# rafaelsoStanford/State_Policy_DiffusionModel

Measured on AMD Instinct MI355X. Metric: denoise-steps/sec (B=4096, horizon=32), higher is better.
Workload: dtype f32 (split-fp16 MFMA operands, fp32 accumulate)

## Files before the change

### include/spdm.h

```cpp
#ifndef SPDM_H
#define SPDM_H

#include <stddef.h>
#include <stdint.h>

#ifdef __cplusplus
extern "C" {
#endif

#define SPDM_NAME_MAX 64
#define SPDM_ABI_VERSION 2

typedef enum {
    SPDM_OK = 0,
    SPDM_ERR_INVALID = -1,
    SPDM_ERR_HIP = -2,
    SPDM_ERR_STATE = -3,
    SPDM_ERR_MISSING = -4,
    SPDM_ERR_NOMEM = -5
} spdm_status;

typedef enum { SPDM_DDPM = 0, SPDM_DDIM = 1 } spdm_scheduler_kind;

typedef struct spdm_handle spdm_handle;
// ... 215 lines not shown
void spdm_decoder_destroy(spdm_decoder* d);

#define SPDM_OPTIM_MAX_SEGMENTS 4
typedef struct { float* d_param; const float* d_grad; float* d_exp_avg; float* d_exp_avg_sq; uint64_t numel; } spdm_optim_segment;
size_t spdm_adam_workspace_doubles(void);
int  spdm_adam_step(int32_t device, const spdm_optim_segment* h_segments, int32_t n_segments, int64_t step,
                    float lr, float beta1, float beta2, float eps, float max_norm,
                    double* d_workspace, void* stream);
size_t spdm_adam_norm_index(void);

int  spdm_debug_geometry(int32_t M, int32_t N, int32_t K, int32_t HW, int32_t W, int32_t taps, uint32_t switches,
                         int32_t out[10]);

int  spdm_debug_whole_tiles(void);

int  spdm_op_gelu(const float* d_x, float* d_y, size_t n, void* stream);

typedef struct {
    int32_t B, H, W, K, N, taps;
    int32_t split;
    int32_t pro;
    int32_t epi;
    const float* d_src;  int32_t src_ld;
    const float* d_skip; int32_t skip_ld;  int32_t up_C;
    const float* h_weight;
    const double* d_src_stats; int32_t src_slots, src_m_tile, src_n_tiles, src_cnorm;
    const float* d_gamma; const float* d_beta;
    const double* d_skip_stats; int32_t skip_slots, skip_m_tile, skip_n_tiles, skip_cnorm;
    const float* d_skip_gamma; const float* d_skip_beta;
    const float* d_bias; const float* d_resid; int32_t resid_ld;
// ... 13 lines not shown
```

### state_policy_diffusionmodel_amd/_lib.py

```python
from __future__ import annotations

import ctypes
import os
from ctypes import POINTER, c_char_p, c_double, c_float, c_int32, c_int64, c_size_t, c_uint64, c_void_p

from .weights import TensorIndex

HERE = os.path.dirname(os.path.abspath(__file__))
LIB_PATH = os.environ.get("SPDM_LIB") or os.path.join(HERE, "libspdm_hip.so")

SPDM_DDPM, SPDM_DDIM = 0, 1
SPDM_FLAG_DEBUG_KEEP = 1
SPDM_FLAG_EXACT_FP32 = 2
SPDM_FLAG_SIMPLE_UNET = 4
SPDM_FLAG_TRAIN = 8
SPDM_FLAG_TRAIN_ATTENTION = 16
SPDM_FLAG_TRAIN_SIMPLE = 32
SPDM_ERR_INVALID = -1
SPDM_ERR_STATE = -3
ABI_VERSION = 2


class SpdmOpGemmArgs(ctypes.Structure):
    _fields_ = ([(n, c_int32) for n in ("B", "H", "W", "K", "N", "taps", "split", "pro", "epi")] +
# ... 95 lines not shown
    "spdm_encoder_update_weights": (c_int32, [c_void_p, c_void_p, c_size_t, c_void_p]),
    "spdm_decoder_create": (c_int32, [c_int32, c_void_p, c_size_t, POINTER(TensorIndex), c_int32, POINTER(c_void_p)]),
    "spdm_decoder_forward": (c_int32, [c_void_p, c_int32, c_void_p, c_void_p, c_void_p]),
    "spdm_decoder_train_loss": (c_int32, [c_void_p, c_int32, c_void_p, c_void_p, c_void_p, c_void_p, c_void_p]),
    "spdm_decoder_backward": (c_int32, [c_void_p, c_int32, c_void_p, c_void_p, c_void_p, c_void_p, c_void_p]),
    "spdm_decoder_update_weights": (c_int32, [c_void_p, c_void_p, c_size_t, c_void_p]),
    "spdm_decoder_destroy": (None, [c_void_p]),
    "spdm_adam_workspace_doubles": (c_size_t, []),
    "spdm_adam_step": (c_int32, [c_int32, POINTER(SpdmOptimSegment), c_int32, c_int64, c_float, c_float, c_float, c_float, c_float,
                                 c_void_p, c_void_p]),
    "spdm_adam_norm_index": (c_size_t, []),
    "spdm_op_gelu": (c_int32, [c_void_p, c_void_p, c_size_t, c_void_p]),
    "spdm_op_gemm": (c_int32, [POINTER(SpdmOpGemmArgs)]),
    "spdm_debug_geometry": (c_int32, [c_int32] * 6 + [ctypes.c_uint32, POINTER(c_int32 * 10)]),
    "spdm_debug_whole_tiles": (c_int32, []),
    "spdm_bench_gemm": (c_int32, [c_int32] * 12 + [POINTER(c_double)]),
}

_lib = None


def load() -> ctypes.CDLL:
    global _lib
    if _lib is not None:
        return _lib
    if not os.path.exists(LIB_PATH):
        raise RuntimeError(
            f"{LIB_PATH} not found: the HIP extension has not been built "
            "(run `python -m state_policy_diffusionmodel_amd.build`); there is no CPU fallback")
    import torch
# ... 19 lines not shown
```

### state_policy_diffusionmodel_amd/csrc/conv_wide.hip

```cpp
#include <algorithm>
#include <cstdlib>

#include "device_utils.h"

namespace spdm {

typedef float f32x16 __attribute__((ext_vector_type(16)));
typedef float f32x4 __attribute__((ext_vector_type(4)));
typedef float f32x2 __attribute__((ext_vector_type(2)));
typedef _Float16 f16x8 __attribute__((ext_vector_type(8)));
typedef _Float16 f16x2 __attribute__((ext_vector_type(2)));

namespace {

constexpr float ACT_SCALE = 16.0f;
constexpr float DESCALE = 1.0f / 2048.0f;
constexpr int CK = 32;
#ifndef WIDE_LDS_PERM
#define WIDE_LDS_PERM 1
#endif
template <bool W2, bool PIPE = false, bool WP = false> struct WidePitch { static constexpr int value = (W2 || PIPE || WP || !WIDE_LDS_PERM) ? 36 : 40; };
constexpr bool wp_active(int t, int rt) { return !((t % 3 == 0 && (rt & 3) == 0) || (t % 3 == 2 && (rt & 3) == 3)); }
constexpr int wp_first(int t) { return (t % 3 == 0) ? 1 : 0; }
constexpr int wp_next(int t, int rt, int RT) {
// ... 5 lines not shown
    int n = 0;
    for (int tt = 0; tt < t; ++tt)
        for (int r = 0; r < RT; ++r) n += wp_active(tt, r) ? 1 : 0;
    for (int r = 0; r < rt; ++r) n += wp_active(t, r) ? 1 : 0;
    return n;
}
#ifndef WIDE_STAGE_GROUP
#define WIDE_STAGE_GROUP 1
#endif
#ifndef WIDE_DB
#define WIDE_DB 0
#endif
#ifndef WIDE_EARLY
#define WIDE_EARLY 0
#endif
#ifndef WIDE_NH
#define WIDE_NH 2
#endif

__device__ __forceinline__ f32x2 split2(float a, float b) {
    unsigned h, l;
    split_pair_f16(a * ACT_SCALE, b * ACT_SCALE, h, l);
    return f32x2{__builtin_bit_cast(float, h), __builtin_bit_cast(float, l)};
}

template <int NT, int PRO, bool W2, int RT, int WN, bool PIPE, bool TWO = false, int WP = 0, bool G2 = false, int WH = 0>
#ifndef WIDE_MINB
#define WIDE_MINB 2
#endif
__global__ __launch_bounds__(256, WIDE_MINB) void conv3x3_wide_kernel(const GemmArgs a, const int epi_slots, const int NS) {
    constexpr int WM = 4 / WN;
    constexpr int CT = 2 * NT;
    constexpr int RW = RT * 16;
    constexpr int NTHR = 256;
    constexpr int RP = NTHR / 8;
    constexpr int M_T = WM * RW, N_T = WN * NT * 32;
    constexpr bool WHOLE = (WH != 0);
    constexpr bool ONE = (WH == 2);
    constexpr int APASS = WHOLE ? M_T / RP : (M_T + 18 + RP - 1) / RP;
    constexpr int FAR = (W2 || WP) ? 4 : 3;
    constexpr int FBR = (NT == 2) ? 2 : 3;
    constexpr int PH = 3 * NT;
    constexpr int BB = (APASS <= 9) ? 7 : (APASS <= 10) ? 6 : 5;
    static_assert(APASS * BB <= 64, "sample-index packing");
    static_assert(!W2 || NT == 2, "the width-2 variant exists for 128-wide tiles");
    static_assert(RT == 8 || (RT == 4 && NT == 2 && !W2), "64-row waves only in the tap-pair loop");
    static_assert(WN == 2 || (WN == 1 && RT == 4), "the 4 x 1 wave arrangement uses 64-row waves");
    static_assert(!TWO || (!PIPE && PRO != PRO_GN_GELU), "two-source input: first conv of a block, plain hand-over");
    static_assert(WP == 0 || WP == 4 || WP == 8, "row permutation for width-4 or width-8 maps");
    static_assert(!WP || (NT == 2 && WN == 2 && !W2 && !PIPE), "row permutation: 128-wide tiles");
    static_assert((16 + 4 * (WP == 8 ? 7 : 6)) % 4 == 0, "A ring phase");
    static_assert(WP != 8 || RT == 8, "width-8 maps: one 128-row block per wave");
    constexpr bool WP8 = (WP == 8);
    constexpr int NI8 = (M_T + 18 + 6) / 8 + 1;
    static_assert(!G2 || (NT == 2 && RT == 4 && !W2 && !PIPE && !WP && !WIDE_DB), "two chunks per hand-over: the plain tap loop, 64 rows per wave");
    static_assert(!WHOLE || (!G2 && !WIDE_DB && !WIDE_EARLY), "whole-sample staging: not in the hand-over experiments");
    extern __shared__ __attribute__((aligned(16))) float smem[];
// ... 24 lines not shown
    float* Abuf = smem;
    float* Awr = smem + (DB ? QZ * LDK : 0);
    float* smean = smem + ((DB || G2) ? 2 : 1) * QZ * LDK;
    float* srstd = smean + NS;

#ifdef SPDM_DIAG
    const bool stamping = (a.debug & DBG_STAMP) && a.stamps != nullptr && tid == 0;
#define WIDE_STAMP(k_) if (stamping) a.stamps[(size_t)bid * 8 + (k_)] = (unsigned long long)__builtin_amdgcn_s_memtime();
    if (stamping) {
        a.stamps[(size_t)bid * 8 + 0] = (unsigned long long)__builtin_amdgcn_s_memrealtime();
        a.stamps[(size_t)bid * 8 + 6] = (unsigned long long)__builtin_amdgcn_s_getreg(63492);
        a.stamps[(size_t)bid * 8 + 7] = (unsigned long long)__builtin_amdgcn_s_getreg(63508);
    }
    const bool dbg_no_mfma = (a.debug & DBG_NO_MFMA) != 0, dbg_no_wload = (a.debug & DBG_NO_WLOAD) != 0;
    const bool dbg_no_aload = (a.debug & DBG_NO_ALOAD) != 0;
#else
#define WIDE_STAMP(k_)
    constexpr bool dbg_no_mfma = false, dbg_no_wload = false, dbg_no_aload = false;
#endif
    WIDE_STAMP(1)
    const int zrow = WP8 ? 8 * NI8 : QA;
    if (tid < LDK) { Abuf[zrow * LDK + tid] = 0.f; Awr[zrow * LDK + tid] = 0.f; }
    if (G2 && tid < LDK) Abuf[(QZ + QA) * LDK + tid] = 0.f;

    constexpr bool pro = (PRO != PRO_NONE);
    constexpr bool pro_gelu = (PRO == PRO_GN_GELU);
    int bh_first = 0;
    float mu1 = 0.f, rs1 = 1.f;
    const int lhw = WHOLE ? __builtin_ctz((unsigned)HW) : 0;
    if constexpr (pro && ONE) {
        sample_mean_rstd(a.pro_stats, m0 / HW, mu1, rs1);
        mu1 = __builtin_bit_cast(float, __builtin_amdgcn_readfirstlane(__builtin_bit_cast(int, mu1)));
        rs1 = __builtin_bit_cast(float, __builtin_amdgcn_readfirstlane(__builtin_bit_cast(int, rs1)));
// ... 55 lines not shown
    const size_t wtap = (size_t)(N >> 4) * 2 * 256;

    f32x4 acc[RT][CT];
#pragma unroll
    for (int rt = 0; rt < RT; ++rt)
#pragma unroll
        for (int ct = 0; ct < CT; ++ct) acc[rt][ct] = f32x4{0.f, 0.f, 0.f, 0.f};

    f32x4 areg[APASS];
    f32x4 g4r = {1.f, 1.f, 1.f, 1.f}, b4r = {0.f, 0.f, 0.f, 0.f};

    int srow_o = srow_t;
#ifdef WIDE_NO_OPAQUE
#define WIDE_OPAQUE_ROW
#else
#define WIDE_OPAQUE_ROW if constexpr (PRO != PRO_NONE && RT == 8) asm volatile("" : "+v"(srow_o));
#endif
#define WIDE_LOAD_A(chunk_) WIDE_LOAD_A_(chunk_, areg, g4r, b4r, ident)
#define WIDE_STAGE_A() WIDE_STAGE_A_(areg, g4r, b4r, ident, Awr)
#define WIDE_LOAD_A_(chunk_, areg_, g4r_, b4r_, ident_)                                              \
    {                                                                                                \
        WIDE_OPAQUE_ROW                                                                              \
        const bool first_ = !TWO || (chunk_) < nc0;                                                  \
        const int cc_ = (TWO && !first_) ? (chunk_) - nc0 : (chunk_);       \
        const float* ab_ = (first_ ? abase : abase1) + cc_ * CK;                                     \
        const int ld_ = first_ ? a.src_ld : a.skip_ld;                                               \
        _Pragma("unroll") for (int p_ = 0; p_ < APASS; ++p_) {                                      \
            const int mc_ = WHOLE ? m0 + p_ * RP + srow_o : min(max(m0 - halo + p_ * RP + srow_o, 0), M - 1); \
            areg_[p_] = *reinterpret_cast<const f32x4*>(ab_ + (size_t)mc_ * ld_);                     \
        }                                                                                            \
        if (pro) {                                                                                   \
// ... 30 lines not shown
                }                                                                                    \
            }                                                                                        \
            if (!WHOLE && !((avalid >> p_) & 1u)) v_ = f32x4{0.f, 0.f, 0.f, 0.f};                       \
            const f32x2 p0_ = split2(v_.x, v_.y), p1_ = split2(v_.z, v_.w);                          \
            {                    \
                const int q_ = p_ * RP + srow_o;                                                     \
                float* row_ = (dst_) + (WHOLE ? (WP8 ? (q_ & 7) * NI8 + (q_ >> 3) : q_) : WP8 ? (q_ < QA ? ((q_ + 7) & 7) * NI8 + ((q_ + 7) >> 3) : 8 * NI8 + 1) : min(q_, QA + 1)) * LDK; \
                *reinterpret_cast<f32x2*>(row_ + c4 * 2) = f32x2{p0_.x, p1_.x};              \
                *reinterpret_cast<f32x2*>(row_ + 16 + c4 * 2) = f32x2{p0_.y, p1_.y};         \
            }                                                                                        \
            if (pro && (p_ % WIDE_STAGE_GROUP) == WIDE_STAGE_GROUP - 1) __builtin_amdgcn_sched_barrier(0);    \
        }                                                                                            \
    }
#define WIDE_LOAD_B(slot_, chunk_, tap_, cp_)                                                        \
    if (!dbg_no_wload) {                                                                             \
        const float* p_ = wfl + (size_t)((tap_) * nchunks + (chunk_)) * wtap + (cp_) * 1024;         \
        _Pragma("unroll") for (int c_ = 0; c_ < 2; ++c_) {                                          \
            fb[slot_][c_][0] = *reinterpret_cast<const f16x8*>(p_ + c_ * 512);                       \
            fb[slot_][c_][1] = *reinterpret_cast<const f16x8*>(p_ + c_ * 512 + 256);                 \
        }                                                                                            \
    }
#define WIDE_LOAD_FA(slot_, tap_, shift_, rt_)                                                       \
    {                                                                                                \
        const unsigned mb_ = (am[(rt_) / 3] >> (9 * ((rt_) % 3) + (tap_))) & 1u;                     \
        const int o_ = mb_ ? aoff0 + WIDE_LDSOFF(rt_) * LDK + (shift_) : zoff;                       \
        fa[slot_][0] = *reinterpret_cast<const f16x8*>(Abuf + o_);                                   \
        fa[slot_][1] = *reinterpret_cast<const f16x8*>(Abuf + o_ + 16);                              \
    }
#define WIDE_STEP(fas_, fbs_, rt_, ct0_)                                                             \
    if (!dbg_no_mfma) {                                                                              \
        acc[rt_][(ct0_)] = __builtin_amdgcn_mfma_f32_16x16x32_f16(fa[fas_][0], fb[fbs_][0][0], acc[rt_][(ct0_)], 0, 0, 0);         \
        acc[rt_][(ct0_) + 1] = __builtin_amdgcn_mfma_f32_16x16x32_f16(fa[fas_][0], fb[fbs_][1][0], acc[rt_][(ct0_) + 1], 0, 0, 0); \
        acc[rt_][(ct0_)] = __builtin_amdgcn_mfma_f32_16x16x32_f16(fa[fas_][0], fb[fbs_][0][1], acc[rt_][(ct0_)], 0, 0, 0);         \
        acc[rt_][(ct0_) + 1] = __builtin_amdgcn_mfma_f32_16x16x32_f16(fa[fas_][0], fb[fbs_][1][1], acc[rt_][(ct0_) + 1], 0, 0, 0); \
        acc[rt_][(ct0_)] = __builtin_amdgcn_mfma_f32_16x16x32_f16(fa[fas_][1], fb[fbs_][0][0], acc[rt_][(ct0_)], 0, 0, 0);         \
        acc[rt_][(ct0_) + 1] = __builtin_amdgcn_mfma_f32_16x16x32_f16(fa[fas_][1], fb[fbs_][1][0], acc[rt_][(ct0_) + 1], 0, 0, 0); \
    }

    const int nrows = (kc1 - kc0) * 3;
    f16x8 fa[FAR][2], fb[FBR][2][2];
#define WIDE_SHIFT(kr_, dwi_) (WP8 ? (((dwi_) - 1) * NI8 + ((kr_) - 1)) * LDK : (((kr_) - 1) * W + ((dwi_) - 1)) * LDK)

    if constexpr (!W2 && NT == 2 && !(WP && RT == 8)) {
        f16x8 fbt[2][4][2], fat[2][2];
#define TAP_LOAD_B(slot_, chunk_, tap_)                                                              \
        if (!dbg_no_wload) {                                                                         \
            const float* p_ = wfl + (size_t)((tap_) * nchunks + (chunk_)) * wtap;                    \
            _Pragma("unroll") for (int c_ = 0; c_ < 4; ++c_) {                                      \
                fbt[slot_][c_][0] = *reinterpret_cast<const f16x8*>(p_ + c_ * 512);                  \
                fbt[slot_][c_][1] = *reinterpret_cast<const f16x8*>(p_ + c_ * 512 + 256);            \
            }                                                                                        \
        }
#define TAP_LOAD_FA(slot_, tap_, shift_, rt_)                                                        \
        {                                                                                            \
            const unsigned mb_ = (am[(rt_) / 3] >> (9 * ((rt_) % 3) + (tap_))) & 1u;                 \
            const int o_ = mb_ ? aoff0 + WIDE_ROWOFF(rt_) * LDK + (shift_) : zoff;                   \
            fat[slot_][0] = *reinterpret_cast<const f16x8*>(Abuf + o_);                              \
            fat[slot_][1] = *reinterpret_cast<const f16x8*>(Abuf + o_ + 16);                         \
        }
        const int TAPS = a.taps;
        const bool t3 = (TAPS == 3);
#define TAP_SHIFT(tap_) (t3 ? ((tap_) - 1) * W * LDK : (((tap_) / 3 - 1) * W + ((tap_) - ((tap_) / 3) * 3 - 1)) * LDK)
// ... 282 lines not shown
                tap = ntap;
                chunk = nchunk;
            }
        }
        }
#undef TAP_LOAD_B
#undef TAP_LOAD_FA
#undef TAP_SHIFT
#undef TAP_BIT
    } else if constexpr (WP) {
#define WP_PLUS(i_) (WP8 ? (i_) : (i_) + (i_) / 3)
#define WP_MINUS(i_) (WP8 ? (i_) + 1 : (i_) + (i_) / 3 + 1)
        constexpr int WS = WP8 ? 7 : 6;
        constexpr int Q1 = 16 + 2 * WS, Q2 = 16 + 4 * WS;
        WIDE_LOAD_B(0, kc0, 1, 0)
        WIDE_LOAD_A(kc0)
        WIDE_STAGE_A()
        __syncthreads();
        WIDE_STAMP(2)
        WIDE_LOAD_FA(0, 1, WIDE_SHIFT(0, 1), 0)
        WIDE_LOAD_FA(1, 1, WIDE_SHIFT(0, 1), 1)
        int chunk = kc0, kr = 0;
        for (int r = 0; r < nrows; ++r) {
            int nkr = kr + 1, nchunk = chunk;
            if (nkr == 3) { nkr = 0; nchunk = chunk + 1; }
            const bool have_next = (r + 1 < nrows);
            const bool next_A = have_next && (nkr == 0);
            const int bkr = have_next ? nkr : kr, bchunk = have_next ? nchunk : chunk;
#pragma unroll
            for (int cp = 0; cp < 2; ++cp) {
                if (cp == 0) { WIDE_LOAD_B(1, chunk, kr * 3 + 1, 1) } else { WIDE_LOAD_B(0, chunk, kr * 3 + 2, 0) }
#pragma unroll
                for (int rt = 0; rt < RT; ++rt) {
                    const int q = cp * 8 + rt;
                    if (q + 2 < 16) { WIDE_LOAD_FA((q + 2) % FAR, kr * 3 + 1, WIDE_SHIFT(kr, 1), (q + 2) % 8) }
                    else { WIDE_LOAD_FA((q + 2) % FAR, kr * 3 + 2, WIDE_SHIFT(kr, 2), WP_PLUS(q + 2 - 16)) }
                    __builtin_amdgcn_sched_barrier(0);
                    WIDE_STEP(q % FAR, cp, rt, cp * 2)
                    __builtin_amdgcn_sched_barrier(0);
                }
            }
#pragma unroll
            for (int cp = 0; cp < 2; ++cp) {
                if (cp == 0) { WIDE_LOAD_B(1, chunk, kr * 3 + 2, 1) } else { WIDE_LOAD_B(0, chunk, kr * 3, 0) }
#pragma unroll
                for (int i = 0; i < WS; ++i) {
                    const int q = 16 + cp * WS + i;
                    if (q + 2 < Q1) { WIDE_LOAD_FA((q + 2) % FAR, kr * 3 + 2, WIDE_SHIFT(kr, 2), WP_PLUS((q + 2 - 16) % WS)) }
                    else { WIDE_LOAD_FA((q + 2) % FAR, kr * 3, WIDE_SHIFT(kr, 0), WP_MINUS(q + 2 - Q1)) }
                    __builtin_amdgcn_sched_barrier(0);
                    WIDE_STEP(q % FAR, cp, WP_PLUS(i), cp * 2)
                    __builtin_amdgcn_sched_barrier(0);
                }
            }
#pragma unroll
            for (int cp = 0; cp < 2; ++cp) {
                if (cp == 0) { WIDE_LOAD_B(1, chunk, kr * 3, 1) } else { WIDE_LOAD_B(0, bchunk, bkr * 3 + 1, 0) }
#pragma unroll
                for (int i = 0; i < WS; ++i) {
                    const int q = Q1 + cp * WS + i;
                    if (q + 2 < Q2) { WIDE_LOAD_FA((q + 2) % FAR, kr * 3, WIDE_SHIFT(kr, 0), WP_MINUS((q + 2 - Q1) % WS)) }
                    else if (have_next && !next_A) { WIDE_LOAD_FA((q + 2) % FAR, nkr * 3 + 1, WIDE_SHIFT(nkr, 1), q + 2 - Q2) }
                    __builtin_amdgcn_sched_barrier(0);
                    WIDE_STEP(q % FAR, cp, WP_MINUS(i), cp * 2)
                    __builtin_amdgcn_sched_barrier(0);
                }
            }
            if (next_A) {
                WIDE_LOAD_A(nchunk)
                __syncthreads();
                WIDE_STAGE_A()
                __syncthreads();
                WIDE_LOAD_FA(0, 1, WIDE_SHIFT(0, 1), 0)
                WIDE_LOAD_FA(1, 1, WIDE_SHIFT(0, 1), 1)
            }
            kr = nkr;
            chunk = nchunk;
        }
#undef WP_PLUS
// ... 35 lines not shown
                }
            }
            if (next_A) {
                WIDE_LOAD_A(nchunk)
                __syncthreads();
                WIDE_STAGE_A()
                __syncthreads();
                WIDE_LOAD_FA(0, 0, WIDE_SHIFT(0, 0), 0)
                WIDE_LOAD_FA(1, 0, WIDE_SHIFT(0, 0), 1)
            }
            kr = nkr;
            chunk = nchunk;
        }
    } else {
        WIDE_LOAD_B(0, kc0, 1, 0)
        WIDE_LOAD_A(kc0)
        WIDE_STAGE_A()
        __syncthreads();
        WIDE_STAMP(2)
        WIDE_LOAD_FA(0, 1, WIDE_SHIFT(0, 1), 0)
        WIDE_LOAD_FA(1, 1, WIDE_SHIFT(0, 1), 1)
        int chunk = kc0, kr = 0;
        for (int r = 0; r < nrows; ++r) {
            int nkr = kr + 1, nchunk = chunk;
            if (nkr == 3) { nkr = 0; nchunk = chunk + 1; }
            const bool have_next = (r + 1 < nrows);
            const bool next_A = have_next && (nkr == 0);
            const int bkr = have_next ? nkr : kr, bchunk = have_next ? nchunk : chunk;
#pragma unroll
            for (int cp = 0; cp < 2; ++cp) {
                if (cp == 0) { WIDE_LOAD_B(1, chunk, kr * 3 + 1, 1) } else { WIDE_LOAD_B(0, chunk, kr * 3 + 2, 0) }
#pragma unroll
                for (int rt = 0; rt < RT; ++rt) {
                    const int q = cp * 8 + rt;
                    if (q + 2 < 16) { WIDE_LOAD_FA((q + 2) % FAR, kr * 3 + 1, WIDE_SHIFT(kr, 1), (q + 2) % 8) }
                    else { WIDE_LOAD_FA((q + 2) % FAR, kr * 3 + 2, WIDE_SHIFT(kr, 2), 2 * (q + 2 - 16)) }
                    __builtin_amdgcn_sched_barrier(0);
                    WIDE_STEP(q % FAR, cp, rt, cp * 2)
                    __builtin_amdgcn_sched_barrier(0);
                }
            }
#pragma unroll
            for (int cp = 0; cp < 2; ++cp) {
                if (cp == 0) { WIDE_LOAD_B(1, chunk, kr * 3 + 2, 1) } else { WIDE_LOAD_B(0, chunk, kr * 3, 0) }
#pragma unroll
                for (int i = 0; i < 4; ++i) {
                    const int q = 16 + cp * 4 + i;
                    if (q + 2 < 24) { WIDE_LOAD_FA((q + 2) % FAR, kr * 3 + 2, WIDE_SHIFT(kr, 2), 2 * ((q + 2 - 16) % 4)) }
                    else { WIDE_LOAD_FA((q + 2) % FAR, kr * 3, WIDE_SHIFT(kr, 0), 2 * (q + 2 - 24) + 1) }
                    __builtin_amdgcn_sched_barrier(0);
                    WIDE_STEP(q % FAR, cp, 2 * i, cp * 2)
                    __builtin_amdgcn_sched_barrier(0);
                }
            }
#pragma unroll
            for (int cp = 0; cp < 2; ++cp) {
                if (cp == 0) { WIDE_LOAD_B(1, chunk, kr * 3, 1) } else { WIDE_LOAD_B(0, bchunk, bkr * 3 + 1, 0) }
#pragma unroll
                for (int i = 0; i < 4; ++i) {
                    const int q = 24 + cp * 4 + i;
                    if (q + 2 < 32) { WIDE_LOAD_FA((q + 2) % FAR, kr * 3, WIDE_SHIFT(kr, 0), 2 * ((q + 2 - 24) % 4) + 1) }
                    else if (have_next && !next_A) { WIDE_LOAD_FA((q + 2) % FAR, nkr * 3 + 1, WIDE_SHIFT(nkr, 1), q + 2 - 32) }
                    __builtin_amdgcn_sched_barrier(0);
                    WIDE_STEP(q % FAR, cp, 2 * i + 1, cp * 2)
                    __builtin_amdgcn_sched_barrier(0);
                }
            }
            if (next_A) {
                WIDE_LOAD_A(nchunk)
                __syncthreads();
                WIDE_STAGE_A()
                __syncthreads();
                WIDE_LOAD_FA(0, 1, WIDE_SHIFT(0, 1), 0)
                WIDE_LOAD_FA(1, 1, WIDE_SHIFT(0, 1), 1)
            }
            kr = nkr;
            chunk = nchunk;
        }
    }
#undef WIDE_LOAD_A
#undef WIDE_STAGE_A
#undef WIDE_LOAD_B
#undef WIDE_LOAD_FA
#undef WIDE_STEP
#undef WIDE_SHIFT
    WIDE_STAMP(3)
    __syncthreads();

#pragma unroll
    for (int rt = 0; rt < RT; ++rt)
#pragma unroll
        for (int ct = 0; ct < CT; ++ct) acc[rt][ct] *= DESCALE;

    const int rb4 = PERM ? ((0x1320 >> (4 * kg)) & 0xF) : kg;
    constexpr int NH = W2 ? 2 : WP ? RT / 4 : WIDE_NH;
    constexpr int HROWS = M_T / NH;
    const bool partial_out = ksp > 1;
// ... 102 lines not shown
#pragma unroll 4
        for (int p = 0; p < HROWS / RPP; ++p) {
            const int lr = p * RPP + r0;
            const int row = m0 + (lr / (RW / NH)) * RW + h * (RW / NH) + lr % (RW / NH);
            if (row < M) {
                const f32x4 v = *reinterpret_cast<const f32x4*>(otile + lr * N_T + c4o * 4);
                *reinterpret_cast<f32x4*>(dstp + (size_t)row * dst_ld + n0 + c4o * 4) = v;
            }
        }
    }
    WIDE_STAMP(5)
#undef WIDE_STAMP
#undef WIDE_ROWOFF
}

template <int NT, int PRO, bool W2 = false, int RT = 8, int WN = 2, bool PIPE = false, bool TWO = false, int WP = 0, bool G2 = false, int WH = 0>
hipError_t launch_wide_cfg(const GemmArgs& a, const GemmGeom& g, hipStream_t s) {
    constexpr int M_T = (4 / WN) * RT * 16, N_T = WN * 32 * NT, NTHR = 256;
    constexpr int APASS = WH ? M_T / 32 : (M_T + 18 + 31) / 32, NSMAX = (APASS <= 9) ? 128 : (APASS <= 10) ? 64 : 32;
    if (WH && (M_T % a.HW != 0 || a.M % M_T != 0 || (WH == 2 && a.HW != M_T))) return hipErrorInvalidValue;
    const int halo = WH ? 0 : a.W + 1;
    const int QA = M_T + 2 * halo;
    const int NS = (((QA - 1) / a.HW + 2) + 3) & ~3;
    if (NS > NSMAX || g.m_tile != M_T || g.n_tile != N_T) return hipErrorInvalidValue;
    constexpr bool DB = PIPE || (WIDE_DB && (NT == 2) && !W2);
    constexpr int LDK = WidePitch<W2, PIPE, (WP != 0) || G2>::value;
    if (PIPE && a.taps != 9) return hipErrorInvalidValue;
    if (WP && (a.taps != 9 || a.W != WP || a.HW % (4 * WP) != 0)) return hipErrorInvalidValue;
    const int QZ = (WP == 8) ? 8 * ((M_T + 18 + 6) / 8 + 1) + 2 : QA + 2;
    size_t lds = (size_t)(((DB || G2) ? 2 : 1) * QZ * LDK + 2 * NS) * sizeof(float);
    lds = std::max(lds, (size_t)((M_T / (W2 ? 2 : WP ? RT / 4 : WIDE_NH)) * N_T + (M_T / 4) * WN * 2) * sizeof(float));
    if (lds > 160 * 1024) return hipErrorInvalidValue;
    auto kern = conv3x3_wide_kernel<NT, PRO, W2, RT, WN, PIPE, TWO, WP, G2, WH>;
    if (hipError_t e = allow_full_lds(reinterpret_cast<const void*>(kern)); e != hipSuccess) return e;
    const int n_mtiles = (a.M + M_T - 1) / M_T;
    if (a.ksplit > 1 && a.K % 64 != 0) return hipErrorInvalidValue;
    if (a.route) *a.route = GemmRoute{ROUTE_WIDE, WP == 4 ? VAR_WP4 : WP == 8 ? VAR_WP8 : W2 ? VAR_W2 : PIPE ? VAR_PIPE : G2 ? VAR_G2 : VAR_PLAIN, M_T, N_T, WH};
    hipLaunchKernelGGL(kern, dim3(n_mtiles * g.n_tiles * std::max(a.ksplit, 1)), dim3(NTHR), lds, s, a, g.slots, NS);
    return hipGetLastError();
}

template <int MODES, int NT, int PRO, bool W2 = false, int RT = 8, int WN = 2, bool PIPE = false, bool TWO = false, int WP = 0>
hipError_t launch_wide_sel(const GemmArgs& a, const GemmGeom& g, hipStream_t s) {
    constexpr int M_T = (4 / WN) * RT * 16;
    const bool whole = !(a.sw & SW_NO_WHOLE_TILES) && M_T % a.HW == 0 && a.M % M_T == 0;
    if constexpr ((MODES & 2) != 0 && PRO != PRO_NONE)
        if (whole && a.HW == M_T) return launch_wide_cfg<NT, PRO, W2, RT, WN, PIPE, TWO, WP, false, 2>(a, g, s);
    if constexpr ((MODES & 1) != 0)
        if (whole) return launch_wide_cfg<NT, PRO, W2, RT, WN, PIPE, TWO, WP, false, 1>(a, g, s);
    return launch_wide_cfg<NT, PRO, W2, RT, WN, PIPE, TWO, WP, false, 0>(a, g, s);
}

}

static bool wide_w2(const GemmArgs& a) { return a.W == 2 && a.taps == 9 && !(a.sw & SW_NO_W2); }

bool conv_wide_supported(const GemmArgs& a, const GemmGeom& g) {
    const bool common = a.split && a.wgt_frag != nullptr && a.W >= 1 && a.W <= 8 && (a.HW & 3) == 0 && a.M % a.HW == 0 &&
                        a.epi == EPI_STATS && a.row_stats == nullptr && a.K % CK == 0 &&
                        (a.debug & ~(DBG_STAMP | DBG_NO_MFMA | DBG_NO_WLOAD | DBG_NO_ALOAD)) == 0 && !(a.sw & SW_NO_WIDE);
    if (!common || a.pro > PRO_GN_GELU) return false;
    if (a.skip != nullptr) {
        if (a.pro == PRO_GN_GELU || a.up_C <= 0 || a.up_C >= a.K || a.up_C % CK != 0 || g.n_tile != 128 || a.skip_ld % 4 != 0 ||
            a.skip_ld < a.K - a.up_C || a.src_ld < a.up_C) return false;
    }
    if (a.ksplit > 1 && a.K % 64 != 0) return false;
    if ((g.m_tile + 2 * (a.W + 1) - 1) / a.HW + 2 > 128) return false;
    if (g.m_tile == 128)
        return g.n_tile == 128 && (a.taps == 9 || (a.taps == 3 && a.W == 1)) && a.K % 64 == 0 && !(a.sw & SW_NO_WIDE128);
    if (g.m_tile != 256) return false;
    if (a.taps == 3) return false;
    if (a.taps != 9 || !(g.n_tile == 128 || g.n_tile == 64)) return false;
    if (wide_w2(a)) return g.n_tile == 128 && (a.HW & 7) == 0;
    if (g.n_tile == 128 && a.K % 64 != 0) return false;
    return true;
// ... 88 lines not shown
```

### state_policy_diffusionmodel_amd/csrc/kernels.h

```cpp
#pragma once
#include <hip/hip_runtime.h>
#include <stdint.h>
#include <mutex>
#include <set>
#include <utility>
#include <vector>

namespace spdm {

inline hipError_t allow_full_lds(const void* kern) {
    static std::mutex mu;
    static std::set<std::pair<int, const void*>> done;
    int dev = 0;
    hipError_t e = hipGetDevice(&dev);
    if (e != hipSuccess) return e;
    std::lock_guard<std::mutex> lk(mu);
    if (done.count({dev, kern})) return hipSuccess;
    e = hipFuncSetAttribute(kern, hipFuncAttributeMaxDynamicSharedMemorySize, (int)(160 * 1024));
    if (e == hipSuccess) done.insert({dev, kern});
    return e;
}

struct StatsRef {
    const double* p;
// ... 28 lines not shown
        {"SPDM_FILM_LOCAL", SW_FILM_LOCAL}, {"SPDM_PIN_GEOMETRY", SW_PIN_GEOMETRY},
        {"SPDM_NO_WP4", SW_NO_WP4}, {"SPDM_G2", SW_G2}, {"SPDM_NO_WP8", SW_NO_WP8},
        {"SPDM_NO_SA_HEAD", SW_NO_SA_HEAD}, {"SPDM_SA_HEAD", SW_SA_HEAD}, {"SPDM_NO_REG64", SW_NO_REG64},
        {"SPDM_NO_SA_CROP", SW_NO_SA_CROP}, {"SPDM_NO_SA_OUTC", SW_NO_SA_OUTC}, {"SPDM_NO_WHOLE_TILES", SW_NO_WHOLE_TILES}};
    *n = (int)(sizeof(t) / sizeof(t[0]));
    return t;
}
unsigned switches_from_env();
int spdm_tune(int idx, int dflt);

enum { PRO_NONE = 0, PRO_GN = 1, PRO_GN_GELU = 2, PRO_POOL = 3, PRO_UPCAT = 4 };
enum { EPI_STATS = 0, EPI_BIAS = 1, EPI_BIAS_GELU = 2, EPI_BIAS_RESID = 3, EPI_PLAIN = 4 };

enum { ROUTE_GEMM = 0, ROUTE_SKINNY = 1, ROUTE_REG = 2, ROUTE_WIDE = 3 };
enum { VAR_PLAIN = 0, VAR_W2 = 1, VAR_WP4 = 2, VAR_WP8 = 3, VAR_PIPE = 4, VAR_G2 = 5 };
struct GemmRoute { int kernel, variant, m_tile, n_tile, whole; };

struct GemmArgs {
    const float* src;  int src_ld;
    const float* wgt;
    int split;
    const float* wgt_frag;
    float* dst;        int dst_ld;
    int M, K, N;
    int geom_M;
    int taps;
    int H, W, HW;
    int pro;  StatsRef pro_stats;  const float* pro_gamma;  const float* pro_beta;
    int up_C;  const float* skip;  int skip_ld;  StatsRef skip_stats;  const float* skip_gamma;  const float* skip_beta;
    int epi;  double* epi_stats;   const float* bias;  const float* resid;  int resid_ld;
    double* row_stats;
    int ksplit;  float* partial;
    unsigned sw;
    int debug;
    unsigned long long* stamps;
    GemmRoute* route;
};
enum { DBG_NO_MFMA = 1, DBG_NO_WLOAD = 2, DBG_NO_GELU = 4, DBG_NO_STORE = 8, DBG_NO_ALOAD = 16, DBG_PP = 64, DBG_STAMP = 128 };

struct GemmGeom {
    int m_tile, n_tile, n_tiles;
    int slots;
    int ksplit;
    int skinny;
    int reg;
    int st_m_tile, st_n_tiles;
};
GemmGeom gemm_geometry(int M, int N, int K, int HW, int W, int taps, int split, unsigned sw, bool stats_epi = false);
GemmGeom gemm_geometry(const GemmArgs& a);
constexpr size_t SPLITK_WORKSPACE_BYTES = (size_t)48 << 20;
__host__ __device__ inline int combine_rows(int HW, int N) {
    int r = HW;
    while ((r & 1) == 0 && (long long)r * N > 2048) r >>= 1;
// ... 283 lines not shown
```

### state_policy_diffusionmodel_amd/csrc/spdm_api.hip

```cpp
#include <hip/hip_runtime.h>

#include <algorithm>
#include <cmath>
#include <cstdarg>
#include <cstdio>
#include <cstdlib>
#include <cstring>
#include <map>
#include <set>
#include <string>
#include <vector>

#include "../../include/spdm.h"
#include "kernels.h"

using namespace spdm;

static thread_local char g_err[512] = "";
static int fail(int code, const char* fmt, ...) {
    va_list ap;
    va_start(ap, fmt);
    vsnprintf(g_err, sizeof(g_err), fmt, ap);
    va_end(ap);
    return code;
// ... 3369 lines not shown
    out[6] = g.st_m_tile; out[7] = g.st_n_tiles;
    out[8] = stats_slots_reserved(HW, N, g.slots);
    out[9] = combine_rows(HW, N);
    return SPDM_OK;
}

extern "C" int spdm_op_gelu(const float* d_x, float* d_y, size_t n, void* stream) {
    if (!d_x || !d_y || n == 0) return fail(SPDM_ERR_INVALID, "bad argument");
    HIP_TRY(launch_gelu(d_x, d_y, n, (hipStream_t)stream));
    if (!stream) HIP_TRY(hipStreamSynchronize(nullptr));
    return SPDM_OK;
}

static int g_op_gemm_whole = -1;
extern "C" int spdm_debug_whole_tiles(void) { return g_op_gemm_whole; }

extern "C" int spdm_op_gemm(spdm_op_gemm_args* p) {
    g_op_gemm_whole = -1;
    if (!p) return fail(SPDM_ERR_INVALID, "op_gemm: null argument");
    spdm_op_gemm_args& q = *p;
    for (int i = 0; i < 10; ++i) q.out[i] = -1;
    const int HW = q.H * q.W;
    if (q.B <= 0 || q.H <= 0 || q.W <= 0 || q.K <= 0 || q.N <= 0) return fail(SPDM_ERR_INVALID, "op_gemm: empty shape");
    if (!(q.taps == 9 || q.taps == 3 || q.taps == 1)) return fail(SPDM_ERR_INVALID, "op_gemm: taps must be 9, 3 or 1");
    if (q.taps == 3 && q.W != 1) return fail(SPDM_ERR_INVALID, "op_gemm: 3-tap convolutions need W == 1");
    if (q.taps == 1 && HW != 1) return fail(SPDM_ERR_INVALID, "op_gemm: a Linear layer has H == W == 1 (B = rows)");
    if (q.taps != 1 && q.W > 8) return fail(SPDM_ERR_INVALID, "op_gemm: maps wider than 8");
    if (q.K % 32 != 0 || q.N % 64 != 0) return fail(SPDM_ERR_INVALID, "op_gemm: K %% 32 == 0 and N %% 64 == 0 required (K %d, N %d)", q.K, q.N);
    if (q.pro < PRO_NONE || q.pro > PRO_UPCAT || q.epi < EPI_STATS || q.epi > EPI_PLAIN) return fail(SPDM_ERR_INVALID, "op_gemm: unknown pro / epi");
    if (!q.d_src || !q.d_dst || !q.h_weight) return fail(SPDM_ERR_INVALID, "op_gemm: src, dst and weight are required");
    if (q.dst_ld < q.N || q.dst_ld % 4 || q.src_ld % 4) return fail(SPDM_ERR_INVALID, "op_gemm: bad leading dimension");
    const bool fused = q.pro == PRO_POOL || q.pro == PRO_UPCAT, two = !fused && q.d_skip != nullptr;
    if (q.src_ld < ((fused && q.pro == PRO_UPCAT) || two ? q.up_C : q.K)) return fail(SPDM_ERR_INVALID, "op_gemm: src_ld too small");
// ... 44 lines not shown
    AffineSrc src{q.d_src, q.src_ld}, skip{q.d_skip, q.skip_ld};
    if (q.d_src_stats)
        src = AffineSrc{q.d_src, q.src_ld, ref(q.d_src_stats, q.src_slots, q.src_m_tile, q.src_n_tiles, src_rows,
                                               q.src_cnorm > 0 ? q.src_cnorm : src_c), q.d_gamma, q.d_beta};
    if (q.d_skip_stats)
        skip = AffineSrc{q.d_skip, q.skip_ld, ref(q.d_skip_stats, q.skip_slots, q.skip_m_tile, q.skip_n_tiles, HW,
                                                  q.skip_cnorm > 0 ? q.skip_cnorm : q.K - q.up_C), q.d_skip_gamma, q.d_skip_beta};
    const int pro = (two && q.d_skip_stats) ? PRO_GN : q.pro;
    GemmArgs a = gemm_args(M, M, q.H, q.W, q.K, q.N, q.taps, split, sw, dp, pro, src, q.up_C, skip, dw,
                           dwf, q.d_dst, q.dst_ld, q.epi, q.epi == EPI_STATS ? q.d_stats : nullptr, q.d_bias,
                           q.d_resid, q.resid_ld, q.d_row_stats);
    if (fused && !gemm_takes_fused_source(a))
        return fail(SPDM_ERR_INVALID, "op_gemm: this launch does not take a fused source (the plan materialises it)");
    if (two && !gemm_takes_two_sources(a))
        return fail(SPDM_ERR_INVALID, "op_gemm: this launch does not take a two-source input (the plan concatenates)");
    GemmRoute r{-1, -1, -1, -1, 0};
    a.route = &r;
    if (q.epi == EPI_STATS) HIP_TRY(hipMemset(q.d_stats, 0xff, (size_t)q.B * g.slots * 2 * sizeof(double)));
    if (q.d_row_stats) HIP_TRY(hipMemset(q.d_row_stats, 0xff, (size_t)M * g.n_tiles * 2 * sizeof(double)));
    const hipError_t el = launch_gemm(a, nullptr);
    const hipError_t es = hipDeviceSynchronize();
    if (el != hipSuccess)
        return fail(el == hipErrorInvalidValue && r.kernel < 0 ? SPDM_ERR_INVALID : SPDM_ERR_HIP,
                    "op_gemm: launch_gemm failed (%s) %s; device: %s", hipGetErrorString(el),
                    r.kernel < 0 ? "before any kernel was dispatched (a host-side shape contract)" : "after a kernel was dispatched",
                    hipGetErrorString(es));
    if (es != hipSuccess) return fail(SPDM_ERR_HIP, "op_gemm: %s", hipGetErrorString(es));
    g_op_gemm_whole = (r.kernel == ROUTE_WIDE) ? r.whole : 0;
    q.out[0] = r.kernel; q.out[1] = r.variant; q.out[2] = r.m_tile; q.out[3] = r.n_tile; q.out[4] = g.ksplit;
    q.out[5] = two ? 1 : 0; q.out[6] = fused ? 1 : 0; q.out[7] = g.slots; q.out[8] = g.st_m_tile; q.out[9] = g.st_n_tiles;
    return SPDM_OK;
}
```

Measured before the change: 506,500.

## Deepen wide-conv weight-fragment ring to three slots for whole-tile W2/WP kernels

Adds a template parameter that lets the wide 3x3 conv kernel keep a three-slot ring of weight (B) fragments instead of two, so weight loads are issued two half-phases ahead of their MFMA use. The aim is to hide global/L2 latency on weight fetches. The deeper ring is enabled by default only for whole-tile, RT=8, width-2 or permuted-pitch variants. It costs extra VGPRs per thread, which may lower occupancy or cause spills. A debug flag that pins weight loads to one hot address and a route query for the ring depth are also added.

```diff
diff --git a/include/spdm.h b/include/spdm.h
--- a/include/spdm.h
+++ b/include/spdm.h
@@ -253,6 +253,8 @@
 
 int  spdm_debug_whole_tiles(void);
 
+int  spdm_debug_weight_ring(void);
+
 int  spdm_op_gelu(const float* d_x, float* d_y, size_t n, void* stream);
 
 typedef struct {
diff --git a/state_policy_diffusionmodel_amd/_lib.py b/state_policy_diffusionmodel_amd/_lib.py
--- a/state_policy_diffusionmodel_amd/_lib.py
+++ b/state_policy_diffusionmodel_amd/_lib.py
@@ -133,6 +133,7 @@
     "spdm_op_gemm": (c_int32, [POINTER(SpdmOpGemmArgs)]),
     "spdm_debug_geometry": (c_int32, [c_int32] * 6 + [ctypes.c_uint32, POINTER(c_int32 * 10)]),
     "spdm_debug_whole_tiles": (c_int32, []),
+    "spdm_debug_weight_ring": (c_int32, []),
     "spdm_bench_gemm": (c_int32, [c_int32] * 12 + [POINTER(c_double)]),
 }
 
diff --git a/state_policy_diffusionmodel_amd/csrc/conv_wide.hip b/state_policy_diffusionmodel_amd/csrc/conv_wide.hip
--- a/state_policy_diffusionmodel_amd/csrc/conv_wide.hip
+++ b/state_policy_diffusionmodel_amd/csrc/conv_wide.hip
@@ -43,6 +43,9 @@
 #ifndef WIDE_EARLY
 #define WIDE_EARLY 0
 #endif
+#ifndef WIDE_FBR
+#define WIDE_FBR 3
+#endif
 #ifndef WIDE_NH
 #define WIDE_NH 2
 #endif
@@ -53,7 +56,7 @@
     return f32x2{__builtin_bit_cast(float, h), __builtin_bit_cast(float, l)};
 }
 
-template <int NT, int PRO, bool W2, int RT, int WN, bool PIPE, bool TWO = false, int WP = 0, bool G2 = false, int WH = 0>
+template <int NT, int PRO, bool W2, int RT, int WN, bool PIPE, bool TWO = false, int WP = 0, bool G2 = false, int WH = 0, int BR = 2>
 #ifndef WIDE_MINB
 #define WIDE_MINB 2
 #endif
@@ -68,8 +71,10 @@
     constexpr bool ONE = (WH == 2);
     constexpr int APASS = WHOLE ? M_T / RP : (M_T + 18 + RP - 1) / RP;
     constexpr int FAR = (W2 || WP) ? 4 : 3;
-    constexpr int FBR = (NT == 2) ? 2 : 3;
+    constexpr int FBR = (NT == 2) ? BR : 3;
+    constexpr int FBD = (NT == 2) ? FBR - 1 : 1;
     constexpr int PH = 3 * NT;
+    static_assert(BR == 2 || BR == 3, "B ring: two or three phases (6 phases per kernel row: slots stay compile-time)");
     constexpr int BB = (APASS <= 9) ? 7 : (APASS <= 10) ? 6 : 5;
     static_assert(APASS * BB <= 64, "sample-index packing");
     static_assert(!W2 || NT == 2, "the width-2 variant exists for 128-wide tiles");
@@ -124,9 +129,10 @@
     }
     const bool dbg_no_mfma = (a.debug & DBG_NO_MFMA) != 0, dbg_no_wload = (a.debug & DBG_NO_WLOAD) != 0;
     const bool dbg_no_aload = (a.debug & DBG_NO_ALOAD) != 0;
+    const bool dbg_hot_wload = (a.debug & DBG_HOT_WLOAD) != 0;
 #else
 #define WIDE_STAMP(k_)
-    constexpr bool dbg_no_mfma = false, dbg_no_wload = false, dbg_no_aload = false;
+    constexpr bool dbg_no_mfma = false, dbg_no_wload = false, dbg_no_aload = false, dbg_hot_wload = false;
 #endif
     WIDE_STAMP(1)
     const int zrow = WP8 ? 8 * NI8 : QA;
@@ -212,7 +218,7 @@
 #ifdef WIDE_NO_OPAQUE
 #define WIDE_OPAQUE_ROW
 #else
-#define WIDE_OPAQUE_ROW if constexpr (PRO != PRO_NONE && RT == 8) asm volatile("" : "+v"(srow_o));
+#define WIDE_OPAQUE_ROW if constexpr ((PRO != PRO_NONE || (W2 && BR == 3)) && RT == 8) asm volatile("" : "+v"(srow_o));
 #endif
 #define WIDE_LOAD_A(chunk_) WIDE_LOAD_A_(chunk_, areg, g4r, b4r, ident)
 #define WIDE_STAGE_A() WIDE_STAGE_A_(areg, g4r, b4r, ident, Awr)
@@ -273,12 +279,24 @@
     }
 #define WIDE_LOAD_B(slot_, chunk_, tap_, cp_)                                                        \
     if (!dbg_no_wload) {                                                                             \
-        const float* p_ = wfl + (size_t)((tap_) * nchunks + (chunk_)) * wtap + (cp_) * 1024;         \
+        const float* p_ = wfl + (size_t)(dbg_hot_wload ? kc0 : (tap_) * nchunks + (chunk_)) * wtap + (cp_) * 1024; \
         _Pragma("unroll") for (int c_ = 0; c_ < 2; ++c_) {                                          \
             fb[slot_][c_][0] = *reinterpret_cast<const f16x8*>(p_ + c_ * 512);                       \
             fb[slot_][c_][1] = *reinterpret_cast<const f16x8*>(p_ + c_ * 512 + 256);                 \
         }                                                                                            \
     }
+#define WIDE_AHEAD_CENTRE(cp_)                                                                       \
+    if constexpr (FBD == 1) { if ((cp_) == 0) { WIDE_LOAD_B(1, chunk, kr * 3 + 1, 1) } else { WIDE_LOAD_B(0, chunk, kr * 3 + 2, 0) } } \
+    else { if ((cp_) == 0) { WIDE_LOAD_B(2, chunk, kr * 3 + 2, 0) } else { WIDE_LOAD_B(0, chunk, kr * 3 + 2, 1) } }
+#define WIDE_AHEAD_PLUS(cp_)                                                                         \
+    if constexpr (FBD == 1) { if ((cp_) == 0) { WIDE_LOAD_B(1, chunk, kr * 3 + 2, 1) } else { WIDE_LOAD_B(0, chunk, kr * 3, 0) } } \
+    else { if ((cp_) == 0) { WIDE_LOAD_B(1, chunk, kr * 3, 0) } else { WIDE_LOAD_B(2, chunk, kr * 3, 1) } }
+#define WIDE_AHEAD_MINUS(cp_)                                                                        \
+    if constexpr (FBD == 1) { if ((cp_) == 0) { WIDE_LOAD_B(1, chunk, kr * 3, 1) } else { WIDE_LOAD_B(0, bchunk, bkr * 3 + 1, 0) } } \
+    else { if ((cp_) == 0) { WIDE_LOAD_B(0, bchunk, bkr * 3 + 1, 0) } else { WIDE_LOAD_B(1, bchunk, bkr * 3 + 1, 1) } }
+#define WIDE_SLOT_CENTRE(cp_) (cp_)
+#define WIDE_SLOT_PLUS(cp_) (FBR == 2 ? (cp_) : 2 - 2 * (cp_))
+#define WIDE_SLOT_MINUS(cp_) (FBR == 2 ? (cp_) : 1 + (cp_))
 #define WIDE_LOAD_FA(slot_, tap_, shift_, rt_)                                                       \
     {                                                                                                \
         const unsigned mb_ = (am[(rt_) / 3] >> (9 * ((rt_) % 3) + (tap_))) & 1u;                     \
@@ -304,7 +322,7 @@
         f16x8 fbt[2][4][2], fat[2][2];
 #define TAP_LOAD_B(slot_, chunk_, tap_)                                                              \
         if (!dbg_no_wload) {                                                                         \
-            const float* p_ = wfl + (size_t)((tap_) * nchunks + (chunk_)) * wtap;                    \
+            const float* p_ = wfl + (size_t)(dbg_hot_wload ? kc0 : (tap_) * nchunks + (chunk_)) * wtap; \
             _Pragma("unroll") for (int c_ = 0; c_ < 4; ++c_) {                                      \
                 fbt[slot_][c_][0] = *reinterpret_cast<const f16x8*>(p_ + c_ * 512);                  \
                 fbt[slot_][c_][1] = *reinterpret_cast<const f16x8*>(p_ + c_ * 512 + 256);            \
@@ -617,6 +635,7 @@
         constexpr int WS = WP8 ? 7 : 6;
         constexpr int Q1 = 16 + 2 * WS, Q2 = 16 + 4 * WS;
         WIDE_LOAD_B(0, kc0, 1, 0)
+        if constexpr (FBD == 2) { WIDE_LOAD_B(1, kc0, 1, 1) }
         WIDE_LOAD_A(kc0)
         WIDE_STAGE_A()
         __syncthreads();
@@ -632,40 +651,40 @@
             const int bkr = have_next ? nkr : kr, bchunk = have_next ? nchunk : chunk;
 #pragma unroll
             for (int cp = 0; cp < 2; ++cp) {
-                if (cp == 0) { WIDE_LOAD_B(1, chunk, kr * 3 + 1, 1) } else { WIDE_LOAD_B(0, chunk, kr * 3 + 2, 0) }
+                WIDE_AHEAD_CENTRE(cp)
 #pragma unroll
                 for (int rt = 0; rt < RT; ++rt) {
                     const int q = cp * 8 + rt;
                     if (q + 2 < 16) { WIDE_LOAD_FA((q + 2) % FAR, kr * 3 + 1, WIDE_SHIFT(kr, 1), (q + 2) % 8) }
                     else { WIDE_LOAD_FA((q + 2) % FAR, kr * 3 + 2, WIDE_SHIFT(kr, 2), WP_PLUS(q + 2 - 16)) }
                     __builtin_amdgcn_sched_barrier(0);
-                    WIDE_STEP(q % FAR, cp, rt, cp * 2)
+                    WIDE_STEP(q % FAR, WIDE_SLOT_CENTRE(cp), rt, cp * 2)
                     __builtin_amdgcn_sched_barrier(0);
                 }
             }
 #pragma unroll
             for (int cp = 0; cp < 2; ++cp) {
-                if (cp == 0) { WIDE_LOAD_B(1, chunk, kr * 3 + 2, 1) } else { WIDE_LOAD_B(0, chunk, kr * 3, 0) }
+                WIDE_AHEAD_PLUS(cp)
 #pragma unroll
                 for (int i = 0; i < WS; ++i) {
                     const int q = 16 + cp * WS + i;
                     if (q + 2 < Q1) { WIDE_LOAD_FA((q + 2) % FAR, kr * 3 + 2, WIDE_SHIFT(kr, 2), WP_PLUS((q + 2 - 16) % WS)) }
                     else { WIDE_LOAD_FA((q + 2) % FAR, kr * 3, WIDE_SHIFT(kr, 0), WP_MINUS(q + 2 - Q1)) }
                     __builtin_amdgcn_sched_barrier(0);
-                    WIDE_STEP(q % FAR, cp, WP_PLUS(i), cp * 2)
+                    WIDE_STEP(q % FAR, WIDE_SLOT_PLUS(cp), WP_PLUS(i), cp * 2)
                     __builtin_amdgcn_sched_barrier(0);
                 }
             }
 #pragma unroll
             for (int cp = 0; cp < 2; ++cp) {
-                if (cp == 0) { WIDE_LOAD_B(1, chunk, kr * 3, 1) } else { WIDE_LOAD_B(0, bchunk, bkr * 3 + 1, 0) }
+                WIDE_AHEAD_MINUS(cp)
 #pragma unroll
                 for (int i = 0; i < WS; ++i) {
                     const int q = Q1 + cp * WS + i;
                     if (q + 2 < Q2) { WIDE_LOAD_FA((q + 2) % FAR, kr * 3, WIDE_SHIFT(kr, 0), WP_MINUS((q + 2 - Q1) % WS)) }
                     else if (have_next && !next_A) { WIDE_LOAD_FA((q + 2) % FAR, nkr * 3 + 1, WIDE_SHIFT(nkr, 1), q + 2 - Q2) }
                     __builtin_amdgcn_sched_barrier(0);
-                    WIDE_STEP(q % FAR, cp, WP_MINUS(i), cp * 2)
+                    WIDE_STEP(q % FAR, WIDE_SLOT_MINUS(cp), WP_MINUS(i), cp * 2)
                     __builtin_amdgcn_sched_barrier(0);
                 }
             }
@@ -731,6 +750,7 @@
         }
     } else {
         WIDE_LOAD_B(0, kc0, 1, 0)
+        if constexpr (FBD == 2) { WIDE_LOAD_B(1, kc0, 1, 1) }
         WIDE_LOAD_A(kc0)
         WIDE_STAGE_A()
         __syncthreads();
@@ -746,40 +766,40 @@
             const int bkr = have_next ? nkr : kr, bchunk = have_next ? nchunk : chunk;
 #pragma unroll
             for (int cp = 0; cp < 2; ++cp) {
-                if (cp == 0) { WIDE_LOAD_B(1, chunk, kr * 3 + 1, 1) } else { WIDE_LOAD_B(0, chunk, kr * 3 + 2, 0) }
+                WIDE_AHEAD_CENTRE(cp)
 #pragma unroll
                 for (int rt = 0; rt < RT; ++rt) {
                     const int q = cp * 8 + rt;
                     if (q + 2 < 16) { WIDE_LOAD_FA((q + 2) % FAR, kr * 3 + 1, WIDE_SHIFT(kr, 1), (q + 2) % 8) }
                     else { WIDE_LOAD_FA((q + 2) % FAR, kr * 3 + 2, WIDE_SHIFT(kr, 2), 2 * (q + 2 - 16)) }
                     __builtin_amdgcn_sched_barrier(0);
-                    WIDE_STEP(q % FAR, cp, rt, cp * 2)
+                    WIDE_STEP(q % FAR, WIDE_SLOT_CENTRE(cp), rt, cp * 2)
                     __builtin_amdgcn_sched_barrier(0);
                 }
             }
 #pragma unroll
             for (int cp = 0; cp < 2; ++cp) {
-                if (cp == 0) { WIDE_LOAD_B(1, chunk, kr * 3 + 2, 1) } else { WIDE_LOAD_B(0, chunk, kr * 3, 0) }
+                WIDE_AHEAD_PLUS(cp)
 #pragma unroll
                 for (int i = 0; i < 4; ++i) {
                     const int q = 16 + cp * 4 + i;
                     if (q + 2 < 24) { WIDE_LOAD_FA((q + 2) % FAR, kr * 3 + 2, WIDE_SHIFT(kr, 2), 2 * ((q + 2 - 16) % 4)) }
                     else { WIDE_LOAD_FA((q + 2) % FAR, kr * 3, WIDE_SHIFT(kr, 0), 2 * (q + 2 - 24) + 1) }
                     __builtin_amdgcn_sched_barrier(0);
-                    WIDE_STEP(q % FAR, cp, 2 * i, cp * 2)
+                    WIDE_STEP(q % FAR, WIDE_SLOT_PLUS(cp), 2 * i, cp * 2)
                     __builtin_amdgcn_sched_barrier(0);
                 }
             }
 #pragma unroll
             for (int cp = 0; cp < 2; ++cp) {
-                if (cp == 0) { WIDE_LOAD_B(1, chunk, kr * 3, 1) } else { WIDE_LOAD_B(0, bchunk, bkr * 3 + 1, 0) }
+                WIDE_AHEAD_MINUS(cp)
 #pragma unroll
                 for (int i = 0; i < 4; ++i) {
                     const int q = 24 + cp * 4 + i;
                     if (q + 2 < 32) { WIDE_LOAD_FA((q + 2) % FAR, kr * 3, WIDE_SHIFT(kr, 0), 2 * ((q + 2 - 24) % 4) + 1) }
                     else if (have_next && !next_A) { WIDE_LOAD_FA((q + 2) % FAR, nkr * 3 + 1, WIDE_SHIFT(nkr, 1), q + 2 - 32) }
                     __builtin_amdgcn_sched_barrier(0);
-                    WIDE_STEP(q % FAR, cp, 2 * i + 1, cp * 2)
+                    WIDE_STEP(q % FAR, WIDE_SLOT_MINUS(cp), 2 * i + 1, cp * 2)
                     __builtin_amdgcn_sched_barrier(0);
                 }
             }
@@ -798,6 +818,12 @@
 #undef WIDE_LOAD_A
 #undef WIDE_STAGE_A
 #undef WIDE_LOAD_B
+#undef WIDE_AHEAD_CENTRE
+#undef WIDE_AHEAD_PLUS
+#undef WIDE_AHEAD_MINUS
+#undef WIDE_SLOT_CENTRE
+#undef WIDE_SLOT_PLUS
+#undef WIDE_SLOT_MINUS
 #undef WIDE_LOAD_FA
 #undef WIDE_STEP
 #undef WIDE_SHIFT
@@ -930,7 +956,7 @@
 #undef WIDE_ROWOFF
 }
 
-template <int NT, int PRO, bool W2 = false, int RT = 8, int WN = 2, bool PIPE = false, bool TWO = false, int WP = 0, bool G2 = false, int WH = 0>
+template <int NT, int PRO, bool W2 = false, int RT = 8, int WN = 2, bool PIPE = false, bool TWO = false, int WP = 0, bool G2 = false, int WH = 0, int BR = 2>
 hipError_t launch_wide_cfg(const GemmArgs& a, const GemmGeom& g, hipStream_t s) {
     constexpr int M_T = (4 / WN) * RT * 16, N_T = WN * 32 * NT, NTHR = 256;
     constexpr int APASS = WH ? M_T / 32 : (M_T + 18 + 31) / 32, NSMAX = (APASS <= 9) ? 128 : (APASS <= 10) ? 64 : 32;
@@ -947,23 +973,27 @@
     size_t lds = (size_t)(((DB || G2) ? 2 : 1) * QZ * LDK + 2 * NS) * sizeof(float);
     lds = std::max(lds, (size_t)((M_T / (W2 ? 2 : WP ? RT / 4 : WIDE_NH)) * N_T + (M_T / 4) * WN * 2) * sizeof(float));
     if (lds > 160 * 1024) return hipErrorInvalidValue;
-    auto kern = conv3x3_wide_kernel<NT, PRO, W2, RT, WN, PIPE, TWO, WP, G2, WH>;
+    auto kern = conv3x3_wide_kernel<NT, PRO, W2, RT, WN, PIPE, TWO, WP, G2, WH, BR>;
     if (hipError_t e = allow_full_lds(reinterpret_cast<const void*>(kern)); e != hipSuccess) return e;
     const int n_mtiles = (a.M + M_T - 1) / M_T;
     if (a.ksplit > 1 && a.K % 64 != 0) return hipErrorInvalidValue;
-    if (a.route) *a.route = GemmRoute{ROUTE_WIDE, WP == 4 ? VAR_WP4 : WP == 8 ? VAR_WP8 : W2 ? VAR_W2 : PIPE ? VAR_PIPE : G2 ? VAR_G2 : VAR_PLAIN, M_T, N_T, WH};
+    if (a.route) *a.route = GemmRoute{ROUTE_WIDE, WP == 4 ? VAR_WP4 : WP == 8 ? VAR_WP8 : W2 ? VAR_W2 : PIPE ? VAR_PIPE : G2 ? VAR_G2 : VAR_PLAIN, M_T, N_T, WH,
+                                       (NT == 2 && RT == 8 && (W2 || WP)) ? BR : 0};
     hipLaunchKernelGGL(kern, dim3(n_mtiles * g.n_tiles * std::max(a.ksplit, 1)), dim3(NTHR), lds, s, a, g.slots, NS);
     return hipGetLastError();
 }
+
+template <bool W2, int RT, int WP, int WH>
+constexpr int wide_bring() { return (WIDE_FBR == 3 && RT == 8 && (W2 || WP) && WH != 0) ? 3 : 2; }
 
 template <int MODES, int NT, int PRO, bool W2 = false, int RT = 8, int WN = 2, bool PIPE = false, bool TWO = false, int WP = 0>
 hipError_t launch_wide_sel(const GemmArgs& a, const GemmGeom& g, hipStream_t s) {
     constexpr int M_T = (4 / WN) * RT * 16;
     const bool whole = !(a.sw & SW_NO_WHOLE_TILES) && M_T % a.HW == 0 && a.M % M_T == 0;
     if constexpr ((MODES & 2) != 0 && PRO != PRO_NONE)
-        if (whole && a.HW == M_T) return launch_wide_cfg<NT, PRO, W2, RT, WN, PIPE, TWO, WP, false, 2>(a, g, s);
+        if (whole && a.HW == M_T) return launch_wide_cfg<NT, PRO, W2, RT, WN, PIPE, TWO, WP, false, 2, wide_bring<W2, RT, WP, 2>()>(a, g, s);
     if constexpr ((MODES & 1) != 0)
-        if (whole) return launch_wide_cfg<NT, PRO, W2, RT, WN, PIPE, TWO, WP, false, 1>(a, g, s);
+        if (whole) return launch_wide_cfg<NT, PRO, W2, RT, WN, PIPE, TWO, WP, false, 1, wide_bring<W2, RT, WP, 1>()>(a, g, s);
     return launch_wide_cfg<NT, PRO, W2, RT, WN, PIPE, TWO, WP, false, 0>(a, g, s);
 }
 
@@ -974,7 +1004,7 @@
 bool conv_wide_supported(const GemmArgs& a, const GemmGeom& g) {
     const bool common = a.split && a.wgt_frag != nullptr && a.W >= 1 && a.W <= 8 && (a.HW & 3) == 0 && a.M % a.HW == 0 &&
                         a.epi == EPI_STATS && a.row_stats == nullptr && a.K % CK == 0 &&
-                        (a.debug & ~(DBG_STAMP | DBG_NO_MFMA | DBG_NO_WLOAD | DBG_NO_ALOAD)) == 0 && !(a.sw & SW_NO_WIDE);
+                        (a.debug & ~(DBG_STAMP | DBG_NO_MFMA | DBG_NO_WLOAD | DBG_NO_ALOAD | DBG_HOT_WLOAD)) == 0 && !(a.sw & SW_NO_WIDE);
     if (!common || a.pro > PRO_GN_GELU) return false;
     if (a.skip != nullptr) {
         if (a.pro == PRO_GN_GELU || a.up_C <= 0 || a.up_C >= a.K || a.up_C % CK != 0 || g.n_tile != 128 || a.skip_ld % 4 != 0 ||
diff --git a/state_policy_diffusionmodel_amd/csrc/kernels.h b/state_policy_diffusionmodel_amd/csrc/kernels.h
--- a/state_policy_diffusionmodel_amd/csrc/kernels.h
+++ b/state_policy_diffusionmodel_amd/csrc/kernels.h
@@ -66,7 +66,7 @@
 
 enum { ROUTE_GEMM = 0, ROUTE_SKINNY = 1, ROUTE_REG = 2, ROUTE_WIDE = 3 };
 enum { VAR_PLAIN = 0, VAR_W2 = 1, VAR_WP4 = 2, VAR_WP8 = 3, VAR_PIPE = 4, VAR_G2 = 5 };
-struct GemmRoute { int kernel, variant, m_tile, n_tile, whole; };
+struct GemmRoute { int kernel, variant, m_tile, n_tile, whole, bring; };
 
 struct GemmArgs {
     const float* src;  int src_ld;
@@ -88,7 +88,7 @@
     unsigned long long* stamps;
     GemmRoute* route;
 };
-enum { DBG_NO_MFMA = 1, DBG_NO_WLOAD = 2, DBG_NO_GELU = 4, DBG_NO_STORE = 8, DBG_NO_ALOAD = 16, DBG_PP = 64, DBG_STAMP = 128 };
+enum { DBG_NO_MFMA = 1, DBG_NO_WLOAD = 2, DBG_NO_GELU = 4, DBG_NO_STORE = 8, DBG_NO_ALOAD = 16, DBG_HOT_WLOAD = 32, DBG_PP = 64, DBG_STAMP = 128 };
 
 struct GemmGeom {
     int m_tile, n_tile, n_tiles;
diff --git a/state_policy_diffusionmodel_amd/csrc/spdm_api.hip b/state_policy_diffusionmodel_amd/csrc/spdm_api.hip
--- a/state_policy_diffusionmodel_amd/csrc/spdm_api.hip
+++ b/state_policy_diffusionmodel_amd/csrc/spdm_api.hip
@@ -3407,9 +3407,11 @@
 
 static int g_op_gemm_whole = -1;
 extern "C" int spdm_debug_whole_tiles(void) { return g_op_gemm_whole; }
+static int g_op_gemm_bring = -1;
+extern "C" int spdm_debug_weight_ring(void) { return g_op_gemm_bring; }
 
 extern "C" int spdm_op_gemm(spdm_op_gemm_args* p) {
-    g_op_gemm_whole = -1;
+    g_op_gemm_whole = g_op_gemm_bring = -1;
     if (!p) return fail(SPDM_ERR_INVALID, "op_gemm: null argument");
     spdm_op_gemm_args& q = *p;
     for (int i = 0; i < 10; ++i) q.out[i] = -1;
@@ -3484,7 +3486,7 @@
         return fail(SPDM_ERR_INVALID, "op_gemm: this launch does not take a fused source (the plan materialises it)");
     if (two && !gemm_takes_two_sources(a))
         return fail(SPDM_ERR_INVALID, "op_gemm: this launch does not take a two-source input (the plan concatenates)");
-    GemmRoute r{-1, -1, -1, -1, 0};
+    GemmRoute r{-1, -1, -1, -1, 0, 0};
     a.route = &r;
     if (q.epi == EPI_STATS) HIP_TRY(hipMemset(q.d_stats, 0xff, (size_t)q.B * g.slots * 2 * sizeof(double)));
     if (q.d_row_stats) HIP_TRY(hipMemset(q.d_row_stats, 0xff, (size_t)M * g.n_tiles * 2 * sizeof(double)));
@@ -3497,6 +3499,7 @@
                     hipGetErrorString(es));
     if (es != hipSuccess) return fail(SPDM_ERR_HIP, "op_gemm: %s", hipGetErrorString(es));
     g_op_gemm_whole = (r.kernel == ROUTE_WIDE) ? r.whole : 0;
+    g_op_gemm_bring = (r.kernel == ROUTE_WIDE) ? r.bring : 0;
     q.out[0] = r.kernel; q.out[1] = r.variant; q.out[2] = r.m_tile; q.out[3] = r.n_tile; q.out[4] = g.ksplit;
     q.out[5] = two ? 1 : 0; q.out[6] = fused ? 1 : 0; q.out[7] = g.slots; q.out[8] = g.st_m_tile; q.out[9] = g.st_n_tiles;
     return SPDM_OK;
```

Result: no change. 507,900 (median of 6 runs) (+0.3%).
